# DVNghiem/genz-tokenize

Hardware: AMD Instinct MI355X
Metric: UTF-8 MB/s tokenized (Tokenize.__call__ hot path: split + BPE + vocab lookup + pad/trunc + mask) (higher is better)
Workload: dtype u8

## Files before the change

genz-tokenize_amd/csrc/gz_api.cpp:

```cpp
#include "../../include/genz_tokenize.h"
#include "gz_kernels.h"

#include <dlfcn.h>
#include <cstdarg>
#include <cstdio>
#include <cstring>
#include <cstdlib>
#include <atomic>
#include <chrono>
#include <mutex>
#include <new>
#include <vector>
#include <unordered_map>
#include <algorithm>
#include <memory>

namespace {

#define g_create_err gz_create_err()

struct DBuf {
    void* p = nullptr;
    size_t cap = 0;
};
// ... 66 lines not shown
        bool small = false, s_dense = true;
        bool small_placed = false;
        int small_G = 0;
        const uint8_t* s_text0 = nullptr; const int64_t* s_off = nullptr; int64_t s_base = 0, s_docs = 0;
        const uint8_t* s_pair0 = nullptr; const int64_t* s_poff = nullptr; int64_t s_pbase = 0;
        int32_t s_max_len = 0; int32_t* s_ids = nullptr; int32_t* s_mask = nullptr; int32_t* s_nreal = nullptr; int32_t* s_arena = nullptr;
        bool keep_words = false;
        int t_slot = 0;
        bool chained = false;
        bool inputs_resident = false;
    } pend;
    hipEvent_t ev[5] = {nullptr, nullptr, nullptr, nullptr, nullptr};
    static constexpr int RING = 1024;
    hipEvent_t ring[RING][2] = {};
    uint64_t ring_n = 0;
    double timing[4] = {0, 0, 0, 0};

    void* comm = nullptr;
    int rank = 0, world = 1;

    DBuf t_words2;
    DBuf t_pair8, t_pair_disp, t_words0p, t_word0_disp;
    DBuf t_pair_hot, t_word_hot;
    struct TextWs { DBuf brk, st, en, blkcnt, docw0, wtok, waux, mtok, mlist, blkmiss, tilecnt, wlist, grpblk, lookback, mq; } tw[2][2];
    uint32_t lb_epoch = 0;
    hipStream_t stream2 = nullptr;
    hipStream_t side = nullptr;
    bool flags_lazy = false;
    bool caller_buffers = false;
    hipEvent_t ev_sf0[2][2] = {}, ev_sf[2][2] = {}, ev_sj[2][2] = {}, ev_sb[2][2] = {};
    hipEvent_t ev_fork = nullptr, ev_join = nullptr;
    hipStream_t xstream = nullptr;
    hipEvent_t ev_tok[4] = {nullptr, nullptr, nullptr, nullptr};
    int32_t* emit_block = nullptr; int32_t emit_bits = 0;
    hipEvent_t ev_blk[4] = {nullptr, nullptr, nullptr, nullptr};
    bool blk_valid[4] = {false, false, false, false};
    hipEvent_t ev_x = nullptr;
    static constexpr int XRING = 64;
    hipEvent_t xring[XRING][2] = {};
    uint64_t xring_n = 0;
    uint64_t enc_seq = 0;
    int x_back = 0;
    bool x_used = false;
    DBuf w_pick, w_rowoff32;
    int64_t* h_pick = nullptr;
    int64_t n_words = 0;
    bool have_dec = false;
    int32_t dec_n_ids = 0;
    size_t dec_bytes_len = 0;
    std::string dec_unk;
    bool dec_unk_set = false;
    DBuf t_dec_entries, t_dec_bytes, w_dec_ids, w_dec_roff, w_dec_rb, w_dec_ooff, w_dec_out;
    DBuf w_pp[2], w_ppoff[2], w_pplen, w_ppaux, w_pp_in, w_pp_inoff, w_ppctl, w_pplen32, w_pplb;
    DBuf w_tiny[8][2];
    hipStream_t s_in = nullptr, s_out = nullptr;
    static constexpr int CSR_SUBS = 16;
    hipEvent_t ev_in[CSR_SUBS] = {}, ev_done[CSR_SUBS] = {};
    DBuf w_csr_ids[2], w_csr_mask[2], w_csr_comp, w_csr_nreal, w_csr_off32;
    uint32_t* h_tot = nullptr;
    uint8_t* h_stage = nullptr; size_t h_stage_cap = 0;
    uint8_t* h_xfer[2] = {nullptr, nullptr}; size_t h_xfer_cap[2] = {0, 0};
    hipEvent_t ev_xfer[2] = {nullptr, nullptr}; bool xfer_busy[2] = {false, false};
    uint8_t* h_tin[2] = {nullptr, nullptr}; size_t h_tin_cap[2] = {0, 0};
    uint8_t* h_cout[3] = {nullptr, nullptr, nullptr}; size_t h_cout_cap[3] = {0, 0, 0};
    DBuf w_stage;
    int cache_status = 0;
// ... 138 lines not shown
void release(DBuf& b) { if (b.p) dev_free(b.p); b.p = nullptr; b.cap = 0; }

}
#include "gz_hostpath.h"
namespace {

template <class V>
int upload(gz_ctx* c, DBuf& b, const V& v)
{
    size_t bytes = v.size() * sizeof(v[0]);
    int rc = ensure(c, b, bytes ? bytes : 16);
    if (rc) return rc;
    return copy_in(c, b.p, v.data(), bytes, c->stream);
}

bool is_dense(const GzShape& S) { return S.pad_mode && S.truncation && S.max_len >= 1; }

GzShape make_shape(int32_t max_len, uint32_t flags)
{
    GzShape S;
    S.max_len = max_len;
    S.pad_mode = (!(flags & GZ_MAX_LEN_NONE) && (flags & GZ_PADDING)) ? 1 : 0;
    S.truncation = (flags & GZ_TRUNCATION) ? 1 : 0;
    return S;
}

static int need_side_streams(gz_ctx* c, bool second)
{
    if (!c->side) HIPCHK(c, hipStreamCreateWithFlags(&c->side, hipStreamNonBlocking));
    if (second && !c->stream2) HIPCHK(c, hipStreamCreateWithFlags(&c->stream2, hipStreamNonBlocking));
    return GZ_OK;
}

int enqueue(gz_ctx* c)
{
    gz_ctx::Pending& p = c->pend;
    hipStream_t s = c->stream;
    const GzDeviceTables* T = (const GzDeviceTables*)c->t_struct.p;
    if (c->x_used) HIPCHK(c, hipStreamWaitEvent(s, c->ev_x, 0));
    const bool no_flags = p.small && !p.ragged;
    const bool lazy_flags = !no_flags && !p.ragged;
    if (!no_flags) {
        if (!p.chained) HIPCHK(c, hipMemsetAsync(c->w_flags.p, 0, 16, s));
        else if (!lazy_flags) HIPCHK(c, hipMemsetAsync((int32_t*)c->w_flags.p + 1, 0, 12, s));
    }
    if (p.timing) {
        hipEvent_t* slot = c->ring[c->ring_n % gz_ctx::RING];
        if (!slot[0]) { HIPCHK(c, hipEventCreate(&slot[0])); HIPCHK(c, hipEventCreate(&slot[1])); }
        HIPCHK(c, hipEventRecord(slot[0], s));
    }
    const bool two = p.subs.size() > 1;
    if (!p.subs.empty()) { int rs = need_side_streams(c, two); if (rs) return rs; }
    if (two) { HIPCHK(c, hipEventRecord(c->ev_fork, s)); HIPCHK(c, hipStreamWaitEvent(c->stream2, c->ev_fork, 0)); }
    if (p.small)
        gz_launch_small(T, p.s_text0, p.s_off, p.s_base, p.s_pair0, p.s_poff, p.s_pbase, p.s_docs, p.small_G, p.s_dense ? 1 : p.small_placed ? 2 : 0, p.s_max_len,
                        p.use_words, p.s_ids, p.s_mask, p.s_nreal, p.s_arena, p.F.row_off, p.F.capacity, (int32_t*)c->w_flags.p + 1, s);
    for (size_t k = 0; k < p.subs.size(); ++k) {
        hipStream_t sk = (k & 1) ? c->stream2 : s;
        const GzAsmArgs& S = p.subs[k];
        for (int tx = 0; tx < S.n_texts; ++tx)
            gz_launch_pipeline_text(c->opt, T, c->dev, S.X[tx], S.n_docs, p.use_words, (int32_t*)c->w_flags.p + 3, sk, c->side, c->ev_sf0[k & 1][tx], c->ev_sf[k & 1][tx], c->ev_sj[k & 1][tx],
                                    p.inputs_resident ? c->ev_sb[k & 1][tx] : nullptr);
        if (p.ragged_direct) gz_launch_rows_ragged(T, S, 0, p.text_bytes, sk);
        else gz_launch_assemble(c->opt, T, S, sk);
    }
    if (two) { HIPCHK(c, hipEventRecord(c->ev_join, c->stream2)); HIPCHK(c, hipStreamWaitEvent(s, c->ev_join, 0)); }
    if (p.timing) { p.t_slot = (int)(c->ring_n % gz_ctx::RING); HIPCHK(c, hipEventRecord(c->ring[p.t_slot][1], s)); c->ring_n++; }
    if (p.emit_block) {
        uint32_t* cur = (uint32_t*)c->w_flags.p + 8 + p.emit_slot;
        {
            uint32_t* off = (uint32_t*)c->w_rowoff32.p;
            if (p.emit_n) HIPCHK(c, hipMemcpyAsync(p.emit_block, p.emit_nreal, (size_t)p.emit_n * 4, hipMemcpyDeviceToDevice, s));
            gz_launch_row_offsets(p.emit_nreal, p.emit_n, off, s);
            gz_launch_compact(p.emit_rows, off, p.emit_n, p.emit_len, p.emit_block + 2 * p.emit_n, p.emit_bits, (uint32_t*)(p.emit_block + p.emit_n), s);
            HIPCHK(c, hipMemcpyAsync(cur, off + p.emit_n, 4, hipMemcpyDeviceToDevice, s));
        }
        HIPCHK(c, hipMemcpyAsync(reinterpret_cast<uint32_t*>(c->h_pick) + 56 + p.emit_slot, cur, 4, hipMemcpyDeviceToHost, s));
        HIPCHK(c, hipEventRecord(c->ev_blk[p.emit_slot], s));
        c->blk_valid[p.emit_slot] = true;
    } else c->blk_valid[c->enc_seq & 3] = false;
    if (p.ragged && !p.small_placed) {
        gz_launch_rowscan(p.F, (int64_t*)c->w_rowlen.p, s);
        if (p.ragged_direct) gz_launch_rows_ragged(T, p.subs[0], 1, p.text_bytes, s);
        else gz_launch_finalize(c->dev, p.F, s);
    }
    if (p.timing && (p.ragged || p.pair)) HIPCHK(c, hipEventRecord(c->ev[2], s));
    if (p.pair) gz_launch_pair(c->dev, p.P, s);
    if (p.timing && (p.ragged || p.pair)) HIPCHK(c, hipEventRecord(c->ev[3], s));
    if (lazy_flags) c->flags_lazy = true;
    else if (!no_flags) { HIPCHK(c, hipMemcpyAsync(c->h_flags, c->w_flags.p, 8, hipMemcpyDeviceToHost, s)); c->flags_lazy = false; }
    else if (!p.chained) c->h_flags[0] = c->h_flags[1] = 0;
    HIPCHK(c, hipEventRecord(c->ev_tok[c->enc_seq & 3], s));
    c->enc_seq++;
    HIPCHK(c, hipGetLastError());
    return GZ_OK;
}

int x_begin(gz_ctx* c)
{
    if (!c->xstream) HIPCHK(c, hipStreamCreateWithFlags(&c->xstream, hipStreamNonBlocking));
    if (c->enc_seq > (uint64_t)c->x_back) HIPCHK(c, hipStreamWaitEvent(c->xstream, c->ev_tok[(c->enc_seq - 1 - (uint64_t)c->x_back) & 3], 0));
    return GZ_OK;
}
int x_end(gz_ctx* c)
{
    HIPCHK(c, hipEventRecord(c->ev_x, c->xstream));
    c->x_used = true;
    return GZ_OK;
}

#ifdef GZ_DIAG
extern "C" int gz_diag_check(unsigned int* out8, int clear);
#endif

int sync_locked(gz_ctx* c)
{
    if (c->flags_lazy) {
        c->flags_lazy = false;
        HIPCHK(c, hipMemcpyAsync(c->h_flags, c->w_flags.p, 8, hipMemcpyDeviceToHost, c->stream));
    }
    HIPCHK(c, hipStreamSynchronize(c->stream));
    if (c->x_used) {
        HIPCHK(c, hipStreamSynchronize(c->xstream));
        int32_t* const bad = reinterpret_cast<int32_t*>(reinterpret_cast<uint8_t*>(c->h_pick) + 384);
        if (*bad) {
            *bad = 0;
            HIPCHK(c, hipMemset((int32_t*)c->w_flags.p + 12, 0, 4));
            c->pend.active = false;
            return fail(c, GZ_E_INVALID, "an exchange block did not fit what was announced for it (a row longer than a row, or entries beyond the block's total): truncated, or written in another layout");
        }
    }
#ifdef GZ_DIAG
    {
        unsigned int e[8] = {0};
// ... 972 lines not shown
try {
    if (!out) return GZ_E_INVALID;
    *out = nullptr;
    static const bool load_timing = getenv("GZ_LOAD_TIMING") != nullptr;
    auto t_last = std::chrono::steady_clock::now();
    auto phase = [&](const char* what) {
        if (!load_timing) return;
        const auto t = std::chrono::steady_clock::now();
        fprintf(stderr, "gz_create: %-38s %7.2f ms\n", what, std::chrono::duration<double, std::milli>(t - t_last).count());
        t_last = t;
    };
    int n = 0;
    hipError_t e = hipGetDeviceCount(&n);
    if (e != hipSuccess || n <= 0)
        return fail(nullptr, GZ_E_NODEVICE, "no HIP device (%s)", e == hipSuccess ? "count is 0" : hipGetErrorString(e));
    if (device_id < 0 || device_id >= n) return fail(nullptr, GZ_E_INVALID, "device %d out of range (0..%d)", device_id, n - 1);
    hipDeviceProp_t prop;
    e = hipGetDeviceProperties(&prop, device_id);
    if (e != hipSuccess) return fail(nullptr, GZ_E_HIP, "hipGetDeviceProperties: %s", hipGetErrorString(e));
    if (std::strncmp(prop.gcnArchName, "gfx950", 6) != 0)
        return fail(nullptr, GZ_E_NODEVICE, "device %d is %s; this library is built for gfx950 only", device_id, prop.gcnArchName);
    phase("device count and properties");
    gz_ctx* c = new (std::nothrow) gz_ctx();
    if (!c) return fail(nullptr, GZ_E_NOMEM, "out of host memory");
    c->device = device_id;
    if (hipSetDevice(device_id) != hipSuccess || hipStreamCreateWithFlags(&c->stream, hipStreamNonBlocking) != hipSuccess ||
        hipHostMalloc((void**)&c->h_flags, 64, hipHostMallocDefault) != hipSuccess) {
        delete c;
        return fail(nullptr, GZ_E_HIP, "stream / pinned memory creation failed");
    }
    std::memset(c->h_flags, 0, 64);
    phase("device, first stream, pinned flags");
    c->opt = gz_default_options();
    for (auto& ev : c->ev) hipEventCreate(&ev);
    hipEventCreateWithFlags(&c->ev_fork, hipEventDisableTiming);
    hipEventCreateWithFlags(&c->ev_join, hipEventDisableTiming);
    for (auto& a : c->ev_sf0) for (auto& e : a) hipEventCreateWithFlags(&e, hipEventDisableTiming);
    for (auto& a : c->ev_sb) for (auto& e : a) hipEventCreateWithFlags(&e, hipEventDisableTiming);
    for (auto& a : c->ev_sf) for (auto& e : a) hipEventCreateWithFlags(&e, hipEventDisableTiming);
    for (auto& a : c->ev_sj) for (auto& e : a) hipEventCreateWithFlags(&e, hipEventDisableTiming);
    for (auto& e : c->ev_tok) hipEventCreateWithFlags(&e, hipEventDisableTiming);
    hipEventCreateWithFlags(&c->ev_x, hipEventDisableTiming);
    phase("streams and events");
    if (hipHostMalloc((void**)&c->h_pick, 512, hipHostMallocDefault) != hipSuccess) { gz_destroy(c); return fail(nullptr, GZ_E_NOMEM, "pinned memory creation failed"); }
    std::memset(c->h_pick, 0, 512);
    phase("pinned pick buffer");
    if (ensure(c, c->w_flags, 64,  true) != GZ_OK) { g_create_err = c->err; gz_destroy(c); return GZ_E_NOMEM; }
    phase("device flags");
    *out = c;
    return GZ_OK;
} GZ_CATCH(nullptr)

void gz_destroy(gz_ctx* c)
try {
    if (!c) return;
    hipSetDevice(c->device);
    for (hipStream_t q : {c->stream, c->stream2, c->side, c->xstream, c->s_in, c->s_out}) if (q) hipStreamSynchronize(q);
    for (gz_bm25* ix : c->bm25_live) delete ix;
    c->bm25_live.clear();
    for (DBuf& b : c->w_bm) release(b);
    if (c->stream2) hipStreamDestroy(c->stream2);
    if (c->ev_fork) hipEventDestroy(c->ev_fork);
    if (c->ev_join) hipEventDestroy(c->ev_join);
    for (auto& e : c->ev_tok) if (e) hipEventDestroy(e);
    for (auto& e : c->ev_blk) if (e) hipEventDestroy(e);
    if (c->ev_x) hipEventDestroy(c->ev_x);
    if (c->xstream) hipStreamDestroy(c->xstream);
    if (c->side) hipStreamDestroy(c->side);
    for (auto& a : c->ev_sf0) for (auto& e : a) if (e) hipEventDestroy(e);
    for (auto& a : c->ev_sb) for (auto& e : a) if (e) hipEventDestroy(e);
    for (auto& a : c->ev_sf) for (auto& e : a) if (e) hipEventDestroy(e);
    for (auto& a : c->ev_sj) for (auto& e : a) if (e) hipEventDestroy(e);
    if (c->s_in) hipStreamDestroy(c->s_in);
    if (c->s_out) hipStreamDestroy(c->s_out);
    for (auto& e : c->ev_in) if (e) hipEventDestroy(e);
// ... 89 lines not shown
    D.words2 = nullptr; D.word2_mask = 0;
    D.pair8 = (const GzPair8*)c->t_pair8.p;
    D.pair_ph = GzPh{(const uint16_t*)c->t_pair_disp.p, H.pair_ph.nbuckets, H.pair_ph.bshift, H.pair_ph.sshift, H.pair_ph.slots - 1, H.pair_ph.k1, H.pair_ph.k2};
    D.words0p = nullptr; D.word0_ph = GzPh{nullptr, 16, 28, 28, 15, 1, 1};
    D.pair_ovf = H.pair_ph.n_overflow; D.word0_ovf = 0;
    D.pair_hot = (const GzPair8*)c->t_pair_hot.p; D.pair_hot_shift = GZ_PAIR_HOT_SHIFT;
    D.word_hot = nullptr;
    if (c->host.enc_words.size() >= (1u << 26)) return fail(c, GZ_E_LIMIT, "vocab has 2^26 or more entries");
    if ((rc = ensure(c, c->t_struct, sizeof(GzDeviceTables)))) return rc;
    { int rcs = copy_in(c, c->t_struct.p, &c->dev, sizeof(GzDeviceTables), c->stream); if (rcs) return rcs; }
    HIPCHK(c, hipStreamSynchronize(c->stream));
    c->have_tables = true;
    phase("upload of the pair / symbol tables");
    if (!hit) {
        rc = build_word_table(c, W);
        if (rc) { c->have_tables = false; return rc; }
        phase("whole-word tables (GPU merge path + perfect hash)");
    }
    rc = install_word_tables(c, W);
    if (rc) { c->have_tables = false; return rc; }
    phase("upload of the whole-word tables");
    if (!hit && !cpath.empty()) {
        bool written = false;
        try { written = cache_write(cdir, cpath, key, c->host, W); } catch (...) {  }
        if (!written) c->cache_status = 4;
        phase("cache write");
    }
    return GZ_OK;
} GZ_CATCH(c)

int gz_debug_set(gz_ctx* c, const char* key, int64_t value)
try {
    int rc;
    if (c) { std::lock_guard<std::mutex> lk(c->mu); rc = gz_option_set(c->opt, key, value); }
    else rc = gz_option_set(gz_default_options(), key, value);
    if (rc) return fail(c, GZ_E_INVALID, "gz_debug_set: unknown key or value out of range: %s = %lld", key ? key : "(null)", (long long)value);
    return GZ_OK;
} GZ_CATCH(c)

int gz_table_cache_status(gz_ctx* c)
try {
    return c ? c->cache_status : GZ_E_INVALID;
} GZ_CATCH(c)

int gz_table_digest(gz_ctx* c, uint8_t out[32])
try {
    if (!c || !out) return GZ_E_INVALID;
    std::lock_guard<std::mutex> lk(c->mu);
    if (!c->have_tables) return fail(c, GZ_E_NOTABLES, "gz_load_tables has not been called");
    HIPCHK(c, hipSetDevice(c->device));
    if (c->pend.active) { int rc = sync_locked(c); if (rc) return rc; }
    Sha256 sha;
    std::vector<uint8_t> buf;
    auto add = [&](const void* dptr, size_t bytes) -> int {
        const uint64_t n = bytes;
        sha.update(&n, 8);
        if (!bytes) return GZ_OK;
        alloc_site(c);
        buf.resize(bytes);
        { int rcs = copy_out(c, buf.data(), dptr, bytes, c->stream); if (rcs) return rcs; }
        sha.update(buf.data(), bytes);
        return GZ_OK;
    };
    const GzDeviceTables& D = c->dev;
    const GzHostTables& H = c->host;
    int rc;
    if ((rc = add(D.merges, (size_t)D.n_ranks * sizeof(GzMergeInfo))) ||
// ... 1103 lines not shown
    return GZ_OK;
} GZ_CATCH(c)

int gz_exchange_select(gz_ctx* c, int back)
try {
    if (!c || back < 0 || back > 2) return c ? fail(c, GZ_E_INVALID, "back must be 0, 1 or 2") : GZ_E_INVALID;
    std::lock_guard<std::mutex> lk(c->mu);
    c->x_back = back;
    return GZ_OK;
} GZ_CATCH(c)

int gz_gather_rows(gz_ctx* c, const int32_t* send_dev, int64_t n_rows_local, int32_t row_len, int32_t* recv_dev,
                   const int64_t* rows_per_rank, int root)
try {
    if (!c) return GZ_E_INVALID;
    std::lock_guard<std::mutex> lk(c->mu);
    if (!c->comm) return fail(c, GZ_E_RCCL, "gz_comm_init has not been called");
    if (root < 0 || root >= c->world || row_len <= 0 || n_rows_local < 0 || !rows_per_rank)
        return fail(c, GZ_E_INVALID, "bad arguments");
    if (rows_per_rank[c->rank] != n_rows_local)
        return fail(c, GZ_E_INVALID, "rows_per_rank[%d] = %lld but n_rows_local = %lld", c->rank,
                    (long long)rows_per_rank[c->rank], (long long)n_rows_local);
    int64_t total_rows = 0;
    for (int q = 0; q < c->world; ++q) {
        if (rows_per_rank[q] < 0) return fail(c, GZ_E_INVALID, "rows_per_rank[%d] is negative", q);
        total_rows += rows_per_rank[q];
    }
    if (n_rows_local > 0 && !send_dev) return fail(c, GZ_E_INVALID, "send_dev is NULL");
    if (c->rank == root && total_rows > 0 && !recv_dev) return fail(c, GZ_E_INVALID, "recv_dev is NULL on the root");
    HIPCHK(c, hipSetDevice(c->device));
    const int ncclInt32 = 2;
    { int rc0 = x_begin(c); if (rc0) return rc0; }
    hipEvent_t* xe = c->xring[c->xring_n % gz_ctx::XRING];
    if (!xe[0]) { HIPCHK(c, hipEventCreate(&xe[0])); HIPCHK(c, hipEventCreate(&xe[1])); }
    HIPCHK(c, hipEventRecord(xe[0], c->xstream));
    if (c->rank == root && n_rows_local > 0) {
        int64_t row0 = 0;
        for (int q = 0; q < root; ++q) row0 += rows_per_rank[q];
        int32_t* dst = recv_dev + row0 * (int64_t)row_len;
        if (dst != send_dev)
            HIPCHK(c, hipMemcpyAsync(dst, send_dev, (size_t)n_rows_local * (size_t)row_len * 4, hipMemcpyDeviceToDevice, c->xstream));
    }
    int r = g_rccl.GroupStart();
    if (r == 0) {
        if (c->rank == root) {
            int64_t row0 = 0;
            for (int q = 0; q < c->world; ++q) {
                const size_t cnt = (size_t)rows_per_rank[q] * (size_t)row_len;
                if (q != root && cnt && r == 0)
                    r = g_rccl.Recv(recv_dev + row0 * (int64_t)row_len, cnt, ncclInt32, q, c->comm, c->xstream);
                row0 += rows_per_rank[q];
            }
        } else {
            const size_t cnt = (size_t)n_rows_local * (size_t)row_len;
            if (cnt) r = g_rccl.Send(send_dev, cnt, ncclInt32, root, c->comm, c->xstream);
        }
        const int r2 = g_rccl.GroupEnd();
        if (r == 0) r = r2;
    }
    if (r != 0)
        return fail(c, GZ_E_RCCL, "RCCL gather failed: %s", g_rccl.GetErrorString ? g_rccl.GetErrorString(r) : "error");
    HIPCHK(c, hipEventRecord(xe[1], c->xstream));
    c->xring_n++;
    { int rc1 = x_end(c); if (rc1) return rc1; }
    return GZ_OK;
} GZ_CATCH(c)

// ... 288 lines not shown
```

genz-tokenize_amd/csrc/gz_common.h:

```cpp
#pragma once
#include <cstdint>
#include <cstdlib>
#include <string>
#include <vector>

#if defined(__HIPCC__)
#include <hip/hip_runtime.h>
#define GZ_HD __host__ __device__ __forceinline__
#else
#define GZ_HD inline
#endif

constexpr uint32_t GZ_MAX_SYMBOLS = (1u << 20) - 2;
constexpr uint32_t GZ_MAX_RANKS   = (1u << 23) - 1;
constexpr uint32_t GZ_SYM_UNKNOWN = 0x80000000u;
constexpr uint32_t GZ_SYM_LASTBIT = 0x40000000u;
constexpr uint32_t GZ_NO_SYMBOL   = 0xFFFFFFFFu;
constexpr uint32_t GZ_RANK_NONE   = 0xFFFFFFFFu;
constexpr uint32_t GZ_PAIR_EMPTY  = 0xFFFFFFFFu;

constexpr int64_t GZ_TEXT_BYTES_LIMIT = 0xFFFF0000ll;
constexpr int64_t GZ_PP_TAIL32_LIMIT = 0xFFFF0000ll;
inline bool gz_pp_tail_is_32bit(int64_t in_bytes) { return in_bytes >= 0 && in_bytes < GZ_PP_TAIL32_LIMIT; }

GZ_HD uint32_t gz_cp_hash(uint32_t cp)
{
    uint32_t h = cp * 0x9E3779B1u;
    return h ^ (h >> 16);
}

#ifndef GZ_TAB_SLACK
#define GZ_TAB_SLACK 16
#endif
struct GzOptions {
    int32_t small = 1;
    int32_t small_wgs = 768;
    int32_t host_direct = 4096;
    int32_t assemble = 3;
    int32_t word_table = 1;
    int32_t pp_fused = 1;
    int32_t sub_batches = 1;
    int32_t docs_per_wave = 0;
    int32_t side = 1;
    int32_t brk_side = 1;
    int64_t scan_multi = 8192;
    int64_t near_limit = 1 << 25;
    int32_t hot_wgs = 0;
    int32_t hot_miss_wgs = 0;
    int64_t m2_split_min = 65536;
    int32_t m2_split_always = 0;
    int32_t tab_slack = GZ_TAB_SLACK;
    int32_t ph_force_overflow = 0;
    int32_t ph_hot_slots = 1024;
    int32_t word_weights = 0;
    int32_t host_threads = 0;
    int32_t dense_csr = 1;
    int32_t host_hints = 0;
    int32_t inject_bad_alloc = 0;
    int32_t bm25_hash_bits = 0;
    int32_t bm25_topk_chunk = 1 << 27;
    int32_t bm25_topk_tile = 0;
    int32_t diag_poison = 0, rows_dpw = 0, rows_dbg = 0, ablate = 0;
    int32_t diag_fresh = 0;
    int32_t diag_fresh_only = -1;
    int32_t diag_exact = 0;
    int32_t diag_guard = 0;
};
GzOptions& gz_default_options();
int gz_option_set(GzOptions& o, const char* key, int64_t value);

inline size_t gz_tab_slack() { return (size_t)gz_default_options().tab_slack; }

constexpr uint32_t GZ_PH_MUL = 0x2C1B3C6Du;
constexpr uint32_t GZ_PH_OVERFLOW = 0xFFFFu;
constexpr uint32_t GZ_PH_LDS_BUCKETS = 16384;
constexpr uint32_t GZ_PAIR_HOT_SLOTS = 4096, GZ_PAIR_HOT_SHIFT = 20;
constexpr uint32_t GZ_WORD_HOT_SLOTS = 1024, GZ_WORD_HOT_SHIFT = 22;
// ... 111 lines not shown
```

genz-tokenize_amd/csrc/gz_host_api.cpp:

```cpp
#include "../../include/genz_tokenize.h"
#include "gz_common.h"

#include <cstring>
#include <new>
#include <string>

std::string& gz_create_err()
{
    static thread_local std::string err;
    return err;
}

GzOptions& gz_default_options()
{
    static GzOptions o;
    return o;
}

int gz_option_set(GzOptions& o, const char* key, int64_t v)
{
    if (!key) return GZ_E_INVALID;
    struct Key { const char* name; int32_t GzOptions::*p32; int64_t GzOptions::*p64; int64_t lo, hi; };
    static const Key keys[] = {
        {"small", &GzOptions::small, nullptr, 0, 1}, {"small_wgs", &GzOptions::small_wgs, nullptr, 1, 1 << 20}, {"host_direct", &GzOptions::host_direct, nullptr, 0, 1 << 20},
        {"assemble", &GzOptions::assemble, nullptr, 1, 3}, {"word_table", &GzOptions::word_table, nullptr, 0, 1},
        {"pp_fused", &GzOptions::pp_fused, nullptr, 0, 1}, {"sub_batches", &GzOptions::sub_batches, nullptr, 1, 8},
        {"docs_per_wave", &GzOptions::docs_per_wave, nullptr, 0, 16}, {"side", &GzOptions::side, nullptr, 0, 1},
        {"brk_side", &GzOptions::brk_side, nullptr, 0, 1}, {"scan_multi", nullptr, &GzOptions::scan_multi, 0, (int64_t)1 << 40},
        {"near_limit", nullptr, &GzOptions::near_limit, 0, 1 << 25}, {"hot_wgs", &GzOptions::hot_wgs, nullptr, 0, 1 << 16},
        {"hot_miss_wgs", &GzOptions::hot_miss_wgs, nullptr, 0, 1 << 16}, {"m2_split_min", nullptr, &GzOptions::m2_split_min, 0, (int64_t)1 << 32},
        {"m2_split_always", &GzOptions::m2_split_always, nullptr, 0, 1},
        {"tab_slack", &GzOptions::tab_slack, nullptr, 2, 64}, {"ph_force_overflow", &GzOptions::ph_force_overflow, nullptr, 0, 1 << 20},
        {"ph_hot_slots", &GzOptions::ph_hot_slots, nullptr, 0, 8192}, {"word_weights", &GzOptions::word_weights, nullptr, 0, 2},
        {"diag_poison", &GzOptions::diag_poison, nullptr, 0, 1}, {"rows_dpw", &GzOptions::rows_dpw, nullptr, 0, 64},
        {"rows_dbg", &GzOptions::rows_dbg, nullptr, 0, 255}, {"ablate", &GzOptions::ablate, nullptr, 0, 1 << 20},
        {"diag_guard", &GzOptions::diag_guard, nullptr, 0, 2}, {"diag_exact", &GzOptions::diag_exact, nullptr, 0, 1}, {"diag_fresh", &GzOptions::diag_fresh, nullptr, 0, 256},
        {"diag_fresh_only", &GzOptions::diag_fresh_only, nullptr, -1, 1 << 20}, {"host_threads", &GzOptions::host_threads, nullptr, 0, 256},
        {"dense_csr", &GzOptions::dense_csr, nullptr, 0, 1}, {"host_hints", &GzOptions::host_hints, nullptr, 0, 3}, {"inject_bad_alloc", &GzOptions::inject_bad_alloc, nullptr, 0, 1 << 30},
        {"bm25_hash_bits", &GzOptions::bm25_hash_bits, nullptr, 0, 62},
        {"bm25_topk_chunk", &GzOptions::bm25_topk_chunk, nullptr, 1, 1 << 30}, {"bm25_topk_tile", &GzOptions::bm25_topk_tile, nullptr, 0, 4096},
    };
    for (const Key& k : keys)
        if (std::strcmp(k.name, key) == 0) {
            if (v < k.lo || v > k.hi) return GZ_E_INVALID;
            if (k.p32) o.*(k.p32) = (int32_t)v; else o.*(k.p64) = v;
            return GZ_OK;
        }
    return GZ_E_INVALID;
}

extern "C" {

#ifdef GZ_HOST_ONLY
int gz_debug_set(gz_ctx*, const char* key, int64_t value)
{
    const int rc = gz_option_set(gz_default_options(), key, value);
    if (rc) gz_create_err() = std::string("gz_debug_set: unknown key or value out of range: ") + (key ? key : "(null)");
    return rc;
}

int gz_version(void) { return GZ_VERSION; }
// ... 91 lines not shown
```

genz-tokenize_amd/csrc/gz_kernels.h:

```cpp
#pragma once
#include "gz_common.h"
#include <hip/hip_runtime.h>

constexpr int GZ_WAVES_PER_BLOCK = 2;
constexpr int GZ_MAX_DOCS_PER_WAVE = 16;
constexpr int32_t GZ_NONE_ = -1;

struct GzShape {
    int32_t max_len;
    int32_t pad_mode;
    int32_t truncation;
};

struct GzFinalizeArgs {
    const int64_t* text_off; const int64_t* pair_off;
    int64_t n_docs;
    GzShape S;
    const int32_t* raw; const int32_t* n_raw;
    int64_t* row_off;
    int64_t capacity;
    int32_t* ids; int32_t* mask; int32_t* n_real;
    int32_t* error_flag;
};

// ... 16 lines not shown
    uint32_t* blkcnt;
    uint32_t* docw0;
    uint32_t* wtok;
    uint32_t* waux;
    uint4* mlist;
    uint32_t* blkmiss;
    uint32_t* grpblk;
    uint32_t* tcnt;
    int64_t wmax;
    uint32_t* ctl;
    uint4* mq;
    uint64_t* lookback;
    uint32_t epoch;
    uint32_t near_lim;
    uint32_t* blklong;
    uint32_t* wlist;
    uint16_t* tilecnt;
    int32_t* mtok;
};

struct GzAsmArgs {
    GzTextBufs X[2];
    int32_t n_texts;
    int64_t n_docs;
    int32_t dense, max_len;
    int32_t* ids; int32_t* mask; int32_t* raw; int32_t* n_real;
    int32_t docs_per_wave;
    const int64_t* row_off; int64_t capacity; int32_t* error_flag;
};

void gz_launch_pipeline_text(const GzOptions& O, const GzDeviceTables* T_dev, const GzDeviceTables& T_host, const GzTextBufs& X, int64_t n_docs, int use_words,
                             int32_t* long_flag , hipStream_t s,
                             hipStream_t side = nullptr, hipEvent_t ev_fork0 = nullptr, hipEvent_t ev_fork = nullptr, hipEvent_t ev_join = nullptr,
                             hipEvent_t ev_brk = nullptr );
void gz_launch_pick(const int64_t* off, const int64_t* off2, int64_t n_docs, int nsub, int64_t* out , hipStream_t s);
void gz_launch_row_offsets(const int32_t* n_real, int64_t n_rows, uint32_t* off, hipStream_t s);
void gz_launch_compact(const int32_t* rows, const uint32_t* off, int64_t n_rows, int32_t row_len, void* out, int bits , uint32_t* first,
                       hipStream_t s);
void gz_launch_expand(const void* compact, int bits, const uint32_t* first, const int32_t* n_real, int64_t n_rows, int32_t row_len, int32_t pad_id,
                      int32_t* ids, int32_t* mask, uint32_t total , int32_t* bad , hipStream_t s);
void gz_launch_assemble(const GzOptions& O, const GzDeviceTables* T_dev, const GzAsmArgs& A, hipStream_t s);
void gz_launch_rows_ragged(const GzDeviceTables* T_dev, const GzAsmArgs& A, int pass, int64_t text_bytes, hipStream_t s);
constexpr int GZ_SMALL_DOC_BYTES = 4096, GZ_SMALL_DOCS_PER_WG = 64;
void gz_launch_small(const GzDeviceTables* T_dev, const uint8_t* text0, const int64_t* off, int64_t base, const uint8_t* pair0, const int64_t* poff,
                     int64_t pbase, int64_t n_docs, int G, int layout , int max_len, int use_words, int32_t* ids,
                     int32_t* mask, int32_t* n_real, int32_t* arena, int64_t* row_off, int64_t capacity, int32_t* error_flag, hipStream_t s);

void gz_launch_rowscan(const GzFinalizeArgs& F, int64_t* row_len_tmp, hipStream_t s);
void gz_launch_finalize(const GzDeviceTables& T, const GzFinalizeArgs& F, hipStream_t s);
void gz_launch_pair(const GzDeviceTables& T, const GzPairArgs& P, hipStream_t s);
void gz_launch_bpe_word(const GzDeviceTables* T_dev, const uint8_t* word, int64_t nbytes, uint32_t* arena,
                        int32_t* out, int32_t cap, int32_t* n_out, hipStream_t s);
void gz_launch_decode(const GzDecTable& D, const int32_t* ids, const int64_t* row_off, int64_t n_rows, int64_t* row_bytes,
                      int64_t* out_off, uint8_t* out, int64_t capacity, hipStream_t s);

struct GzPpArgs {
    const uint8_t* in; const int64_t* in_off;
    const int64_t* in_len;
    int32_t in_abs;
    int64_t n_docs;
    uint8_t* out;
    int64_t* out_len;
    int64_t* aux;
    int32_t op;
    int64_t skip_upto;
};
struct GzPpFusedArgs {
// ... 132 lines not shown
```

genz-tokenize_amd/csrc/gz_pipeline.inc:

```

namespace {

#if defined(GZ_DIAG) || defined(GZ_ABLATE)
constexpr bool GZ_DIAG_ON = true;
#else
constexpr bool GZ_DIAG_ON = false;
#endif
constexpr int PBLK = 4096;
#ifndef GZ_PWPB
#define GZ_PWPB 4
#endif
constexpr int PWPB = GZ_PWPB;
constexpr uint32_t W_MISS = 0x80000000u;
constexpr uint32_t W_PEND = 0x40000000u;
constexpr uint32_t W_LONG = 0x20000000u;
constexpr uint32_t W_HUGE = 0x10000000u;
constexpr uint32_t W_NEAR = 0x20000000u;
constexpr uint32_t W_NEAR_MAX = 1u << 25;
__device__ __forceinline__ const int32_t* miss_pieces(const GzTextBufs& X, uint32_t rec, uint32_t w)
{
#ifdef GZ_DIAG
    const uint64_t place = (rec & W_NEAR) ? (uint64_t)X.B + 32u + (rec & (W_NEAR_MAX - 1u)) : (uint64_t)X.waux[w];
    const uint64_t cnt = (rec & W_NEAR) ? ((rec >> 25) & 15u) + 1u : (rec & 0x0FFFFFFFu);
    if (!(GZ_CHK(501, (rec & W_PEND) ? 1 : 0, 1) && GZ_CHK(502, place + cnt, 2 * (X.B + 32) + 1))) return X.mtok;
// ... 595 lines not shown
                while (rem) {
                    const uint64_t low = rem & (0 - rem);
                    pick |= low;
                    rem &= ~(low | (low << 1));
                }
            }
            const uint32_t prow = (uint32_t)(pick >> sh) & RM;
            const bool picked = (prow >> k) & 1u;
            const bool consumed = ((prow << 1) >> k) & 1u;
            const bool keep = rv && k < n && !consumed;
            const uint32_t krow = (uint32_t)(wballot(keep) >> sh) & RM;
            if (keep) S[__popc(krow & ((1u << k) - 1u))] = picked ? merged : s;
            n -= __popc(prow);
        }
        if (rv) {
            if (k < n) X.mtok[start + k] = token_id(T, S[k], k == n - 1);
            if (k == 0) X.wtok[widx] = W_MISS | (uint32_t)n;
        }
        const bool ov = mv && over && k == 0;
        const uint64_t ob = wballot(ov);
        if (ob) {
            uint32_t base = 0;
            if (lane == 0) base = atomicAdd(X.wlist, (uint32_t)__popcll(ob));
            base = (uint32_t)__builtin_amdgcn_readfirstlane((int)base);
            if (ov) { X.wtok[widx] = rec | W_LONG; X.wlist[1 + base + below(ob)] = widx; }
            nover = 1;
        }
    }
    return nover;
}

}

__global__ __launch_bounds__(WAVE * PWPB) __attribute__((amdgpu_waves_per_eu(8, 8))) void gz_miss_wide_kernel(const GzDeviceTables* __restrict__ Tp, GzTextBufs X, int32_t* long_flag, int lds_disp)
{
    __shared__ MissLds lds[PWPB];
    extern __shared__ __attribute__((aligned(16))) uint8_t wide_dyn[];
    const int lane = lane_id();
    const uint32_t n = X.wlist[0];
    const uint32_t wave = blockIdx.x * PWPB + threadIdx.x / WAVE, nwaves = gridDim.x * PWPB;
    if (blockIdx.x * PWPB * 2u >= n) return;
    const GzDeviceTables T = *Tp;
    uint16_t* ldisp = nullptr;
    if (lds_disp) {
        ldisp = reinterpret_cast<uint16_t*>(wide_dyn);
        const uint4* src = reinterpret_cast<const uint4*>(T.pair_ph.disp);
        for (uint32_t i = threadIdx.x; i < T.pair_ph.nbuckets / 8u; i += blockDim.x) reinterpret_cast<uint4*>(ldisp)[i] = src[i];
        __syncthreads();
    }
    if (wave * 2u >= n) return;
    MissLds& L = lds[threadIdx.x / WAVE];
    for (uint32_t i = wave * 2u; i < n; i += nwaves * 2u) {
        const int nq = (int)min(2u, n - i);
        if (lane < nq) L.q[1][lane] = X.wlist[1 + i + lane];
        const int n64 = merge_passes<32, 1>(T, L, X, nq, lane, 0, long_flag, ldisp);
        if (n64) merge_passes<64, 2>(T, L, X, n64, lane, 0, long_flag, ldisp);
    }
}

__global__ __launch_bounds__(WAVE * PWPB) void gz_long_kernel(const GzDeviceTables* __restrict__ Tp, GzTextBufs X, const int32_t* long_flag)
{
    __shared__ uint32_t lsym[PWPB][PLONG];
    if (*long_flag == 0) return;
    const int lane = lane_id();
    const uint32_t n = X.ctl[0];
    for (uint32_t i = blockIdx.x * PWPB + threadIdx.x / WAVE; i < n; i += gridDim.x * PWPB) {
        if (!GZ_CHK(411, i, X.wmax + 6)) continue;
        const uint32_t lw = X.wlist[X.wmax + 6 - (int64_t)i];
        if (!GZ_CHK(412, lw, X.wmax)) continue;
        const uint32_t lrec = X.wtok[lw];
        if ((lrec & (W_MISS | W_PEND | W_HUGE)) != (W_MISS | W_PEND | W_HUGE)) continue;
        const uint32_t lstart = X.waux[lw];
        if (!GZ_CHK(413, lstart, X.B)) continue;
        int64_t lnb = lrec & 0x7FFFu;
        if (lnb == 0x7FFF)
            lnb = scan_word_end(X, (int64_t)lstart + 1) - lstart;
        Emit E;
        E.ids = X.mtok + lstart; E.mask = nullptr; E.symout = nullptr; E.pad_hit = nullptr;
        E.limit = 0x7FFFFFFF; E.stop = 0x7FFFFFFF; E.ntok = 0; E.pad_id = 0x7FFFFFFF;
        const int nt = long_word(Tp, lsym[threadIdx.x / WAVE], PLONG, X.tb + lstart, lnb, (lrec & 0x8000u) != 0,
                                 reinterpret_cast<uint32_t*>(X.mtok + lstart), E, lane);
        if (lane == 0) X.wtok[lw] = W_MISS | (uint32_t)nt;
    }
}

namespace {
struct AsmLds {
    uint32_t dw[GMAX + 1];
    int32_t doc_ntok[GMAX];
    int64_t row_base[GMAX];
    uint8_t pad_hit[GMAX];
};
}

__global__ __launch_bounds__(WAVE * PWPB) void gz_assemble_kernel(const GzDeviceTables* __restrict__ Tp, GzAsmArgs A)
// ... 618 lines not shown
{
    if (n_rows >= 8 * SC32) {
        hipLaunchKernelGGL(gz_scan32x_local_kernel, dim3((unsigned)(n_rows / SC32 + 1)), dim3(1024), 0, s, n_real, n_rows, off);
        hipLaunchKernelGGL(gz_scan32x_bases_kernel, dim3(1), dim3(1024), 0, s, off, n_rows);
        hipLaunchKernelGGL(gz_scan32x_add_kernel, dim3((unsigned)(n_rows / 256 + 1)), dim3(256), 0, s, off, n_rows);
        return;
    }
    if (n_rows > 0) hipLaunchKernelGGL(gz_copy_counts_kernel, dim3((unsigned)((n_rows + 255) / 256)), dim3(256), 0, s, n_real, n_rows, off);
    hipLaunchKernelGGL(gz_scan32_kernel, dim3(1), dim3(1024), 0, s, off, n_rows, (uint32_t*)nullptr);
}

void gz_launch_compact(const int32_t* rows, const uint32_t* off, int64_t n_rows, int32_t row_len, void* out, int bits, uint32_t* first, hipStream_t s)
{
    if (n_rows <= 0) return;
    const dim3 grid((unsigned)((n_rows + PWPB * CK - 1) / (PWPB * CK))), block(WAVE * PWPB);
    if (bits == 16) hipLaunchKernelGGL(gz_compact_kernel<uint16_t>, grid, block, 0, s, rows, off, n_rows, row_len, (uint16_t*)out, first);
    else hipLaunchKernelGGL(gz_compact_kernel<int32_t>, grid, block, 0, s, rows, off, n_rows, row_len, (int32_t*)out, first);
}

void gz_launch_expand(const void* compact, int bits, const uint32_t* first, const int32_t* n_real, int64_t n_rows, int32_t row_len, int32_t pad_id,
                      int32_t* ids, int32_t* mask, uint32_t total, int32_t* bad, hipStream_t s)
{
    if (n_rows <= 0) return;
    const dim3 grid((unsigned)((n_rows + PWPB - 1) / PWPB)), block(WAVE * PWPB);
    if (bits == 16) hipLaunchKernelGGL(gz_expand_kernel<uint16_t>, grid, block, 0, s, (const uint16_t*)compact, first, n_real, n_rows, row_len, pad_id, ids, mask, total, bad);
    else hipLaunchKernelGGL(gz_expand_kernel<int32_t>, grid, block, 0, s, (const int32_t*)compact, first, n_real, n_rows, row_len, pad_id, ids, mask, total, bad);
}

void gz_launch_hot_words(const GzOptions& O, const GzDeviceTables* T, const GzDeviceTables& Th, const GzTextBufs& X, int use_words, hipStream_t s);
void gz_launch_hot_pre(const GzDeviceTables* T, const GzDeviceTables& Th, const GzTextBufs& X, int use_words, hipStream_t s);
void gz_launch_hot_miss(const GzOptions& O, const GzDeviceTables* T, const GzDeviceTables& Th, const GzTextBufs& X, int use_words, hipStream_t s);

void gz_launch_pipeline_text(const GzOptions& O, const GzDeviceTables* T, const GzDeviceTables& Th, const GzTextBufs& X, int64_t n_docs, int use_words, int32_t* long_flag,
                             hipStream_t s, hipStream_t side, hipEvent_t ev_fork0, hipEvent_t ev_fork, hipEvent_t ev_join, hipEvent_t ev_brk)
{
    const int fork_side = O.side;
    bool par0 = false;
    const size_t bm_bytes = (size_t)((X.B + TILE) / TILE) * (TILE / 8) + 64;
    const int brk_on = O.brk_side;
    const bool brk_side = brk_on && fork_side && side && ev_fork0 && ev_fork && ev_join && ev_brk;
    hipStream_t sb = brk_side ? side : s;
    hipMemsetAsync(X.brk, 0, bm_bytes, sb);
    if (n_docs > 1)
        hipLaunchKernelGGL(gz_brk_kernel, dim3((unsigned)((n_docs + 255) / 256)), dim3(256), 0, sb, X.off, n_docs,
                           reinterpret_cast<uint32_t*>(X.brk));
    hipMemsetAsync(X.blklong, 0, (size_t)(X.ctl + 65 - X.blklong) * 4, sb);
    if (brk_side) { hipEventRecord(ev_brk, side); hipStreamWaitEvent(s, ev_brk, 0); }
    const unsigned nb = (unsigned)((X.nblk + PWPB - 1) / PWPB);
    const int64_t scan_multi = O.scan_multi;
    auto scan32 = [&](uint32_t* v, uint32_t* grp, int which) {
        if (X.nblk < scan_multi)
            hipLaunchKernelGGL(gz_scan32_kernel, dim3(1), dim3(1024), 0, s, v, X.nblk, grp);
        else
            hipLaunchKernelGGL(gz_scan32m_kernel, dim3((unsigned)((X.nblk + SCH) / SCH)), dim3(256), 0, s, v, X.nblk, grp,
                               reinterpret_cast<unsigned long long*>(X.lookback), X.ctl + 2 + which, X.epoch + 1u + (uint32_t)which, long_flag - 3);
    };
    if (!(GZ_DIAG_ON && (use_words & 0x100))) {
        hipLaunchKernelGGL(gz_classify_kernel, dim3(nb), dim3(WAVE * PWPB), 0, s, X);
        scan32(X.blkcnt, nullptr, 0);
    }
    par0 = fork_side && side && ev_fork0 && ev_fork && ev_join;
    if (par0) {
        hipEventRecord(ev_fork0, s); hipStreamWaitEvent(side, ev_fork0, 0);
        hipLaunchKernelGGL(gz_docw0_kernel, dim3((unsigned)((n_docs + 1 + 255) / 256)), dim3(256), 0, side, X, n_docs);
    } else hipLaunchKernelGGL(gz_docw0_kernel, dim3((unsigned)((n_docs + 1 + 255) / 256)), dim3(256), 0, s, X, n_docs);
    gz_launch_hot_words(O, T, Th, X, use_words, s);
    scan32(X.blkmiss, X.grpblk, 1);
    auto wide = [&](hipStream_t q) {
        const int ldw = Th.pair_ph.nbuckets <= GZ_PH_LDS_BUCKETS ? 1 : 0;
        hipLaunchKernelGGL(gz_miss_wide_kernel, dim3(nb < 2048u ? nb : 2048u), dim3(WAVE * PWPB), ldw ? (size_t)Th.pair_ph.nbuckets * 2 : 0, q, T, X, long_flag, ldw);
        hipLaunchKernelGGL(gz_long_kernel, dim3(nb < 1024u ? nb : 1024u), dim3(WAVE * PWPB), 0, q, T, X, (const int32_t*)long_flag);
    };
    gz_launch_hot_pre(T, Th, X, use_words, s);
    const bool par = fork_side && side && ev_fork && ev_join;
    if (par) {
        hipEventRecord(ev_fork, s); hipStreamWaitEvent(side, ev_fork, 0);
        wide(side);
        hipEventRecord(ev_join, side);
    }
    gz_launch_hot_miss(O, T, Th, X, use_words, s);
    if (par) hipStreamWaitEvent(s, ev_join, 0);
    else wide(s);
}

void gz_launch_rows_ragged(const GzDeviceTables* T, const GzAsmArgs& A0, int pass, int64_t text_bytes, hipStream_t s)
{
    GzAsmArgs A = A0;
    if (A.n_docs <= 0) return;
    const int64_t avg = text_bytes / A.n_docs;
    const bool big = avg > 1024;
    A.docs_per_wave = big ? 1 : 8;
    const int64_t waves = (A.n_docs + A.docs_per_wave - 1) / A.docs_per_wave;
    const int64_t blocks = (waves + PWPB - 1) / PWPB;
    if (big) {
        if (pass == 0) hipLaunchKernelGGL((gz_rowsr_kernel<1536, false>), dim3((unsigned)blocks), dim3(WAVE * PWPB), 0, s, T, A);
        else hipLaunchKernelGGL((gz_rowsr_kernel<1536, true>), dim3((unsigned)blocks), dim3(WAVE * PWPB), 0, s, T, A);
    } else {
        if (pass == 0) hipLaunchKernelGGL((gz_rowsr_kernel<512, false>), dim3((unsigned)blocks), dim3(WAVE * PWPB), 0, s, T, A);
        else hipLaunchKernelGGL((gz_rowsr_kernel<512, true>), dim3((unsigned)blocks), dim3(WAVE * PWPB), 0, s, T, A);
    }
}

void gz_launch_assemble(const GzOptions& O, const GzDeviceTables* T, const GzAsmArgs& A0, hipStream_t s)
{
// ... 50 lines not shown
```

Measured before the change: 298,300.

## Use device-scope non-timing events, skip unneeded token events, prioritize side-stream tail kernels

Recreates all ordering events with hipEventDisableSystemFence (device scope) and timing disabled where not needed, through a new make_events helper. The per-call ev_tok record is skipped unless an exchange or emit path needs it, and x_begin records it lazily when required. Side-stream miss_wide and long kernels now raise wave priority via s_setprio so they finish sooner while running alongside the main-stream hot_miss work. An optional late timing stamp is added but is off by default. The aim is to cut event and fence overhead and shorten the critical path, at the cost of more complex event bookkeeping.

```diff
diff --git a/genz-tokenize_amd/csrc/gz_api.cpp b/genz-tokenize_amd/csrc/gz_api.cpp
--- a/genz-tokenize_amd/csrc/gz_api.cpp
+++ b/genz-tokenize_amd/csrc/gz_api.cpp
@@ -122,6 +122,7 @@
     hipEvent_t ev_fork = nullptr, ev_join = nullptr;
     hipStream_t xstream = nullptr;
     hipEvent_t ev_tok[4] = {nullptr, nullptr, nullptr, nullptr};
+    uint64_t tok_seq[4] = {0, 0, 0, 0};
     int32_t* emit_block = nullptr; int32_t emit_bits = 0;
     hipEvent_t ev_blk[4] = {nullptr, nullptr, nullptr, nullptr};
     bool blk_valid[4] = {false, false, false, false};
@@ -326,6 +327,41 @@
     return GZ_OK;
 }
 
+constexpr unsigned GZ_EV_DEVICE = hipEventDisableSystemFence;
+unsigned order_flags(const gz_ctx* c, bool timed)
+{
+    return (timed ? 0u : (unsigned)hipEventDisableTiming) | (c->opt.ev_scope ? GZ_EV_DEVICE : 0u);
+}
+int timed_pair(gz_ctx* c, hipEvent_t* pr)
+{
+    if (!pr[0]) { HIPCHK(c, hipEventCreateWithFlags(&pr[0], order_flags(c, true))); HIPCHK(c, hipEventCreateWithFlags(&pr[1], order_flags(c, true))); }
+    return GZ_OK;
+}
+void drop_events(gz_ctx* c)
+{
+    auto drop = [](hipEvent_t& e) { if (e) hipEventDestroy(e); e = nullptr; };
+    for (auto& e : c->ev) drop(e);
+    drop(c->ev_fork); drop(c->ev_join); drop(c->ev_x);
+    for (auto& e : c->ev_tok) drop(e);
+    for (auto* a : {c->ev_sf0, c->ev_sb, c->ev_sf, c->ev_sj}) for (int k = 0; k < 2; ++k) for (int t = 0; t < 2; ++t) drop(a[k][t]);
+    for (auto& pr : c->ring) { drop(pr[0]); drop(pr[1]); }
+    for (auto& pr : c->xring) { drop(pr[0]); drop(pr[1]); }
+    c->ring_n = 0; c->xring_n = 0;
+    for (auto& q : c->tok_seq) q = 0;
+}
+int make_events(gz_ctx* c)
+{
+    drop_events(c);
+    for (auto& e : c->ev) HIPCHK(c, hipEventCreateWithFlags(&e, order_flags(c, true)));
+    const unsigned f = order_flags(c, false);
+    HIPCHK(c, hipEventCreateWithFlags(&c->ev_fork, f));
+    HIPCHK(c, hipEventCreateWithFlags(&c->ev_join, f));
+    for (auto* a : {c->ev_sf0, c->ev_sb, c->ev_sf, c->ev_sj}) for (int k = 0; k < 2; ++k) for (int t = 0; t < 2; ++t) HIPCHK(c, hipEventCreateWithFlags(&a[k][t], f));
+    for (auto& e : c->ev_tok) HIPCHK(c, hipEventCreateWithFlags(&e, f));
+    HIPCHK(c, hipEventCreateWithFlags(&c->ev_x, f));
+    return GZ_OK;
+}
+
 int enqueue(gz_ctx* c)
 {
     gz_ctx::Pending& p = c->pend;
@@ -333,6 +369,7 @@
     const GzDeviceTables* T = (const GzDeviceTables*)c->t_struct.p;
     if (c->x_used) HIPCHK(c, hipStreamWaitEvent(s, c->ev_x, 0));
     const bool no_flags = p.small && !p.ragged;
+    hipEvent_t stamp = nullptr;
     const bool lazy_flags = !no_flags && !p.ragged;
     if (!no_flags) {
         if (!p.chained) HIPCHK(c, hipMemsetAsync(c->w_flags.p, 0, 16, s));
@@ -340,8 +377,9 @@
     }
     if (p.timing) {
         hipEvent_t* slot = c->ring[c->ring_n % gz_ctx::RING];
-        if (!slot[0]) { HIPCHK(c, hipEventCreate(&slot[0])); HIPCHK(c, hipEventCreate(&slot[1])); }
-        HIPCHK(c, hipEventRecord(slot[0], s));
+        { int re = timed_pair(c, slot); if (re) return re; }
+        if (c->opt.stamp_late && !p.small && !p.subs.empty() && p.subs[0].n_texts > 0) stamp = slot[0];
+        else HIPCHK(c, hipEventRecord(slot[0], s));
     }
     const bool two = p.subs.size() > 1;
     if (!p.subs.empty()) { int rs = need_side_streams(c, two); if (rs) return rs; }
@@ -354,7 +392,7 @@
         const GzAsmArgs& S = p.subs[k];
         for (int tx = 0; tx < S.n_texts; ++tx)
             gz_launch_pipeline_text(c->opt, T, c->dev, S.X[tx], S.n_docs, p.use_words, (int32_t*)c->w_flags.p + 3, sk, c->side, c->ev_sf0[k & 1][tx], c->ev_sf[k & 1][tx], c->ev_sj[k & 1][tx],
-                                    p.inputs_resident ? c->ev_sb[k & 1][tx] : nullptr);
+                                    p.inputs_resident ? c->ev_sb[k & 1][tx] : nullptr, k == 0 && tx == 0 ? stamp : nullptr);
         if (p.ragged_direct) gz_launch_rows_ragged(T, S, 0, p.text_bytes, sk);
         else gz_launch_assemble(c->opt, T, S, sk);
     }
@@ -384,7 +422,10 @@
     if (lazy_flags) c->flags_lazy = true;
     else if (!no_flags) { HIPCHK(c, hipMemcpyAsync(c->h_flags, c->w_flags.p, 8, hipMemcpyDeviceToHost, s)); c->flags_lazy = false; }
     else if (!p.chained) c->h_flags[0] = c->h_flags[1] = 0;
-    HIPCHK(c, hipEventRecord(c->ev_tok[c->enc_seq & 3], s));
+    if (!c->opt.ev_tok || c->x_used || p.emit_block) {
+        HIPCHK(c, hipEventRecord(c->ev_tok[c->enc_seq & 3], s));
+        c->tok_seq[c->enc_seq & 3] = c->enc_seq + 1;
+    }
     c->enc_seq++;
     HIPCHK(c, hipGetLastError());
     return GZ_OK;
@@ -393,7 +434,11 @@
 int x_begin(gz_ctx* c)
 {
     if (!c->xstream) HIPCHK(c, hipStreamCreateWithFlags(&c->xstream, hipStreamNonBlocking));
-    if (c->enc_seq > (uint64_t)c->x_back) HIPCHK(c, hipStreamWaitEvent(c->xstream, c->ev_tok[(c->enc_seq - 1 - (uint64_t)c->x_back) & 3], 0));
+    if (c->enc_seq > (uint64_t)c->x_back) {
+        const uint64_t call = c->enc_seq - 1 - (uint64_t)c->x_back;
+        if (c->tok_seq[call & 3] != call + 1) { HIPCHK(c, hipEventRecord(c->ev_tok[call & 3], c->stream)); c->tok_seq[call & 3] = call + 1; }
+        HIPCHK(c, hipStreamWaitEvent(c->xstream, c->ev_tok[call & 3], 0));
+    }
     return GZ_OK;
 }
 int x_end(gz_ctx* c)
@@ -1432,15 +1477,7 @@
     std::memset(c->h_flags, 0, 64);
     phase("device, first stream, pinned flags");
     c->opt = gz_default_options();
-    for (auto& ev : c->ev) hipEventCreate(&ev);
-    hipEventCreateWithFlags(&c->ev_fork, hipEventDisableTiming);
-    hipEventCreateWithFlags(&c->ev_join, hipEventDisableTiming);
-    for (auto& a : c->ev_sf0) for (auto& e : a) hipEventCreateWithFlags(&e, hipEventDisableTiming);
-    for (auto& a : c->ev_sb) for (auto& e : a) hipEventCreateWithFlags(&e, hipEventDisableTiming);
-    for (auto& a : c->ev_sf) for (auto& e : a) hipEventCreateWithFlags(&e, hipEventDisableTiming);
-    for (auto& a : c->ev_sj) for (auto& e : a) hipEventCreateWithFlags(&e, hipEventDisableTiming);
-    for (auto& e : c->ev_tok) hipEventCreateWithFlags(&e, hipEventDisableTiming);
-    hipEventCreateWithFlags(&c->ev_x, hipEventDisableTiming);
+    if (make_events(c) != GZ_OK) { g_create_err = c->err; gz_destroy(c); return GZ_E_HIP; }
     phase("streams and events");
     if (hipHostMalloc((void**)&c->h_pick, 512, hipHostMallocDefault) != hipSuccess) { gz_destroy(c); return fail(nullptr, GZ_E_NOMEM, "pinned memory creation failed"); }
     std::memset(c->h_pick, 0, 512);
@@ -1596,7 +1633,20 @@
 int gz_debug_set(gz_ctx* c, const char* key, int64_t value)
 try {
     int rc;
-    if (c) { std::lock_guard<std::mutex> lk(c->mu); rc = gz_option_set(c->opt, key, value); }
+    if (c) {
+        std::lock_guard<std::mutex> lk(c->mu);
+        const int32_t scope = c->opt.ev_scope;
+        rc = gz_option_set(c->opt, key, value);
+        if (!rc && c->opt.ev_scope != scope) {
+            c->opt.ev_scope = scope;
+            HIPCHK(c, hipSetDevice(c->device));
+            int rs = sync_locked(c);
+            if (rs) return rs;
+            for (hipStream_t q : {c->stream, c->stream2, c->side, c->xstream, c->s_in, c->s_out}) if (q) HIPCHK(c, hipStreamSynchronize(q));
+            c->opt.ev_scope = (int32_t)value;
+            return make_events(c);
+        }
+    }
     else rc = gz_option_set(gz_default_options(), key, value);
     if (rc) return fail(c, GZ_E_INVALID, "gz_debug_set: unknown key or value out of range: %s = %lld", key ? key : "(null)", (long long)value);
     return GZ_OK;
@@ -2766,7 +2816,7 @@
     const int ncclInt32 = 2;
     { int rc0 = x_begin(c); if (rc0) return rc0; }
     hipEvent_t* xe = c->xring[c->xring_n % gz_ctx::XRING];
-    if (!xe[0]) { HIPCHK(c, hipEventCreate(&xe[0])); HIPCHK(c, hipEventCreate(&xe[1])); }
+    { int re = timed_pair(c, xe); if (re) return re; }
     HIPCHK(c, hipEventRecord(xe[0], c->xstream));
     if (c->rank == root && n_rows_local > 0) {
         int64_t row0 = 0;
diff --git a/genz-tokenize_amd/csrc/gz_common.h b/genz-tokenize_amd/csrc/gz_common.h
--- a/genz-tokenize_amd/csrc/gz_common.h
+++ b/genz-tokenize_amd/csrc/gz_common.h
@@ -43,6 +43,10 @@
     int32_t docs_per_wave = 0;
     int32_t side = 1;
     int32_t brk_side = 1;
+    int32_t ev_scope = 1;
+    int32_t ev_tok = 1;
+    int32_t stamp_late = 0;
+    int32_t side_tail = 1;
     int64_t scan_multi = 8192;
     int64_t near_limit = 1 << 25;
     int32_t hot_wgs = 0;
diff --git a/genz-tokenize_amd/csrc/gz_host_api.cpp b/genz-tokenize_amd/csrc/gz_host_api.cpp
--- a/genz-tokenize_amd/csrc/gz_host_api.cpp
+++ b/genz-tokenize_amd/csrc/gz_host_api.cpp
@@ -26,7 +26,8 @@
         {"assemble", &GzOptions::assemble, nullptr, 1, 3}, {"word_table", &GzOptions::word_table, nullptr, 0, 1},
         {"pp_fused", &GzOptions::pp_fused, nullptr, 0, 1}, {"sub_batches", &GzOptions::sub_batches, nullptr, 1, 8},
         {"docs_per_wave", &GzOptions::docs_per_wave, nullptr, 0, 16}, {"side", &GzOptions::side, nullptr, 0, 1},
-        {"brk_side", &GzOptions::brk_side, nullptr, 0, 1}, {"scan_multi", nullptr, &GzOptions::scan_multi, 0, (int64_t)1 << 40},
+        {"brk_side", &GzOptions::brk_side, nullptr, 0, 1}, {"ev_scope", &GzOptions::ev_scope, nullptr, 0, 1}, {"ev_tok", &GzOptions::ev_tok, nullptr, 0, 1},
+        {"side_tail", &GzOptions::side_tail, nullptr, 0, 1}, {"stamp_late", &GzOptions::stamp_late, nullptr, 0, 1}, {"scan_multi", nullptr, &GzOptions::scan_multi, 0, (int64_t)1 << 40},
         {"near_limit", nullptr, &GzOptions::near_limit, 0, 1 << 25}, {"hot_wgs", &GzOptions::hot_wgs, nullptr, 0, 1 << 16},
         {"hot_miss_wgs", &GzOptions::hot_miss_wgs, nullptr, 0, 1 << 16}, {"m2_split_min", nullptr, &GzOptions::m2_split_min, 0, (int64_t)1 << 32},
         {"m2_split_always", &GzOptions::m2_split_always, nullptr, 0, 1},
diff --git a/genz-tokenize_amd/csrc/gz_kernels.h b/genz-tokenize_amd/csrc/gz_kernels.h
--- a/genz-tokenize_amd/csrc/gz_kernels.h
+++ b/genz-tokenize_amd/csrc/gz_kernels.h
@@ -72,7 +72,8 @@
 void gz_launch_pipeline_text(const GzOptions& O, const GzDeviceTables* T_dev, const GzDeviceTables& T_host, const GzTextBufs& X, int64_t n_docs, int use_words,
                              int32_t* long_flag , hipStream_t s,
                              hipStream_t side = nullptr, hipEvent_t ev_fork0 = nullptr, hipEvent_t ev_fork = nullptr, hipEvent_t ev_join = nullptr,
-                             hipEvent_t ev_brk = nullptr );
+                             hipEvent_t ev_brk = nullptr ,
+                             hipEvent_t ev_stamp = nullptr );
 void gz_launch_pick(const int64_t* off, const int64_t* off2, int64_t n_docs, int nsub, int64_t* out , hipStream_t s);
 void gz_launch_row_offsets(const int32_t* n_real, int64_t n_rows, uint32_t* off, hipStream_t s);
 void gz_launch_compact(const int32_t* rows, const uint32_t* off, int64_t n_rows, int32_t row_len, void* out, int bits , uint32_t* first,
diff --git a/genz-tokenize_amd/csrc/gz_pipeline.inc b/genz-tokenize_amd/csrc/gz_pipeline.inc
--- a/genz-tokenize_amd/csrc/gz_pipeline.inc
+++ b/genz-tokenize_amd/csrc/gz_pipeline.inc
@@ -651,10 +651,12 @@
 
 }
 
+template <bool PRIO>
 __global__ __launch_bounds__(WAVE * PWPB) __attribute__((amdgpu_waves_per_eu(8, 8))) void gz_miss_wide_kernel(const GzDeviceTables* __restrict__ Tp, GzTextBufs X, int32_t* long_flag, int lds_disp)
 {
     __shared__ MissLds lds[PWPB];
     extern __shared__ __attribute__((aligned(16))) uint8_t wide_dyn[];
+    if (PRIO) __builtin_amdgcn_s_setprio(3);
     const int lane = lane_id();
     const uint32_t n = X.wlist[0];
     const uint32_t wave = blockIdx.x * PWPB + threadIdx.x / WAVE, nwaves = gridDim.x * PWPB;
@@ -677,9 +679,11 @@
     }
 }
 
+template <bool PRIO>
 __global__ __launch_bounds__(WAVE * PWPB) void gz_long_kernel(const GzDeviceTables* __restrict__ Tp, GzTextBufs X, const int32_t* long_flag)
 {
     __shared__ uint32_t lsym[PWPB][PLONG];
+    if (PRIO) __builtin_amdgcn_s_setprio(3);
     if (*long_flag == 0) return;
     const int lane = lane_id();
     const uint32_t n = X.ctl[0];
@@ -1364,7 +1368,7 @@
 void gz_launch_hot_miss(const GzOptions& O, const GzDeviceTables* T, const GzDeviceTables& Th, const GzTextBufs& X, int use_words, hipStream_t s);
 
 void gz_launch_pipeline_text(const GzOptions& O, const GzDeviceTables* T, const GzDeviceTables& Th, const GzTextBufs& X, int64_t n_docs, int use_words, int32_t* long_flag,
-                             hipStream_t s, hipStream_t side, hipEvent_t ev_fork0, hipEvent_t ev_fork, hipEvent_t ev_join, hipEvent_t ev_brk)
+                             hipStream_t s, hipStream_t side, hipEvent_t ev_fork0, hipEvent_t ev_fork, hipEvent_t ev_join, hipEvent_t ev_brk, hipEvent_t ev_stamp)
 {
     const int fork_side = O.side;
     bool par0 = false;
@@ -1378,6 +1382,7 @@
                            reinterpret_cast<uint32_t*>(X.brk));
     hipMemsetAsync(X.blklong, 0, (size_t)(X.ctl + 65 - X.blklong) * 4, sb);
     if (brk_side) { hipEventRecord(ev_brk, side); hipStreamWaitEvent(s, ev_brk, 0); }
+    if (ev_stamp) hipEventRecord(ev_stamp, s);
     const unsigned nb = (unsigned)((X.nblk + PWPB - 1) / PWPB);
     const int64_t scan_multi = O.scan_multi;
     auto scan32 = [&](uint32_t* v, uint32_t* grp, int which) {
@@ -1400,8 +1405,16 @@
     scan32(X.blkmiss, X.grpblk, 1);
     auto wide = [&](hipStream_t q) {
         const int ldw = Th.pair_ph.nbuckets <= GZ_PH_LDS_BUCKETS ? 1 : 0;
-        hipLaunchKernelGGL(gz_miss_wide_kernel, dim3(nb < 2048u ? nb : 2048u), dim3(WAVE * PWPB), ldw ? (size_t)Th.pair_ph.nbuckets * 2 : 0, q, T, X, long_flag, ldw);
-        hipLaunchKernelGGL(gz_long_kernel, dim3(nb < 1024u ? nb : 1024u), dim3(WAVE * PWPB), 0, q, T, X, (const int32_t*)long_flag);
+        const bool prio = O.side_tail && q != s;
+        const dim3 gw(nb < 2048u ? nb : 2048u), gl(nb < 1024u ? nb : 1024u), blk(WAVE * PWPB);
+        const size_t dyn = ldw ? (size_t)Th.pair_ph.nbuckets * 2 : 0;
+        if (prio) {
+            hipLaunchKernelGGL(gz_miss_wide_kernel<true>, gw, blk, dyn, q, T, X, long_flag, ldw);
+            hipLaunchKernelGGL(gz_long_kernel<true>, gl, blk, 0, q, T, X, (const int32_t*)long_flag);
+        } else {
+            hipLaunchKernelGGL(gz_miss_wide_kernel<false>, gw, blk, dyn, q, T, X, long_flag, ldw);
+            hipLaunchKernelGGL(gz_long_kernel<false>, gl, blk, 0, q, T, X, (const int32_t*)long_flag);
+        }
     };
     gz_launch_hot_pre(T, Th, X, use_words, s);
     const bool par = fork_side && side && ev_fork && ev_join;
```

After: 296,500. Within noise of the previous version (-0.6%).
